# CESNET/UltraGrid

Measured on NVIDIA H100. Metric: 7680x4320 frames/sec encode (UYVY->DXT1), higher is better.
Workload: dtype f32

## Files before the change

include/ugb200.h:

```cpp
#ifndef UGB200_H
#define UGB200_H

#include "cuda_wrapper.h"

#ifdef __cplusplus
extern "C" {
#endif

enum ugb200_codec {
        UGB_VIDEO_CODEC_NONE = 0,
        UGB_RGBA, UGB_UYVY, UGB_YUYV, UGB_VUYA, UGB_R10k, UGB_R12L, UGB_v210, UGB_DVS10, UGB_DXT1, UGB_DXT1_YUV,
        UGB_DXT5, UGB_RGB, UGB_JPEG, UGB_JPEG_XS, UGB_RAW, UGB_H264, UGB_H265, UGB_VP8, UGB_VP9, UGB_BGR, UGB_J2K,
        UGB_J2KR, UGB_HW_VDPAU, UGB_HFYU, UGB_FFV1, UGB_CFHD, UGB_RG48, UGB_AV1, UGB_I420, UGB_Y216, UGB_Y416,
        UGB_PRORES, UGB_PRORES_4444, UGB_PRORES_4444_XQ, UGB_PRORES_422_HQ, UGB_PRORES_422, UGB_PRORES_422_PROXY,
        UGB_PRORES_422_LT, UGB_APV, UGB_PYROWAVE, UGB_DRM_PRIME,
        UGB_VIDEO_CODEC_COUNT
};


UGB_API int ugb200_rgb_to_dxt1_async(const void *src, void *out, int size_x, int size_y, cuda_wrapper_stream_t stream);
UGB_API int ugb200_yuv_to_dxt1_async(const void *src, void *out, int size_x, int size_y, cuda_wrapper_stream_t stream);
UGB_API int ugb200_rgb_to_dxt6_async(const void *src, void *out, int size_x, int size_y, cuda_wrapper_stream_t stream);
UGB_API int ugb200_yuv_to_dxt6_async(const void *src, void *out, int size_x, int size_y, cuda_wrapper_stream_t stream);

UGB_API int ugb200_uyvy_to_dxt1_async(const void *src, void *out, int size_x, int size_y, long src_pitch,
                              cuda_wrapper_stream_t stream);
UGB_API int ugb200_uyvy_to_dxt6_async(const void *src, void *out, int size_x, int size_y, long src_pitch,
                              cuda_wrapper_stream_t stream);

UGB_API int ugb200_pixfmt_supported(int in_codec, int out_codec);
UGB_API int ugb200_pixfmt_convert(int in_codec, int out_codec, void *dst, long dst_pitch, const void *src, long src_pitch,
                          int dst_len, int height, long src_size, int rshift, int gshift, int bshift,
                          cuda_wrapper_stream_t stream);

UGB_API int ugb200_pixfmt_staged_mode(int mode);

enum ugb200_line_func {
        UGB_LINE_ABGR_TO_RGB = 1,
        UGB_LINE_BGRA_TO_RGB,
        UGB_LINE_TO_RGBA_INPLACE,
        UGB_LINE_UYVY_TO_GRAYSCALE,
};
UGB_API int ugb200_vc_copyline(int func, void *dst, long dst_pitch, const void *src, long src_pitch, int dst_len, int height, long src_size,
                               int rshift, int gshift, int bshift, cuda_wrapper_stream_t stream);

UGB_API int ugb200_dxt1_to_rgb(const void *src, void *out, int w, int h, long out_pitch, int bgr, cuda_wrapper_stream_t stream);
UGB_API int ugb200_dxt5ycocg_to_rgb(const void *src, void *out, int w, int h, long out_pitch, int bgr, cuda_wrapper_stream_t stream);

struct ugb200_to_planar_data {
        int            width;
        int            height;
        unsigned char *out_data[4];
        unsigned       out_linesize[4];
        const unsigned char *in_data;
};
UGB_API int ugb200_v210_to_p010le(const struct ugb200_to_planar_data *d, long in_linesize, cuda_wrapper_stream_t stream);
UGB_API int ugb200_y216_to_p010le(const struct ugb200_to_planar_data *d, cuda_wrapper_stream_t stream);
UGB_API int ugb200_uyvy_to_nv12(const struct ugb200_to_planar_data *d, cuda_wrapper_stream_t stream);
UGB_API int ugb200_rgba_to_bgra(const struct ugb200_to_planar_data *d, cuda_wrapper_stream_t stream);
UGB_API int ugb200_vuya_to_i444(const struct ugb200_to_planar_data *d, cuda_wrapper_stream_t stream);
UGB_API int ugb200_uyvy_to_i420(const struct ugb200_to_planar_data *d, cuda_wrapper_stream_t stream);
UGB_API int ugb200_r12l_to_gbrp12le(const struct ugb200_to_planar_data *d, cuda_wrapper_stream_t stream);
UGB_API int ugb200_r12l_to_gbrp16le(const struct ugb200_to_planar_data *d, cuda_wrapper_stream_t stream);
UGB_API int ugb200_r12l_to_rgbp12le(const struct ugb200_to_planar_data *d, cuda_wrapper_stream_t stream);

struct ugb200_from_planar_data {
        int            width;
        int            height;
        unsigned char *out_data;
        unsigned       out_pitch;
        const unsigned char *in_data[4];
        unsigned       in_linesize[4];
        int            in_depth;
        int            log2_chroma_h;
        int            rgb_shift[3];
};
UGB_API int ugb200_gbrap_to_rgb(const struct ugb200_from_planar_data *d, cuda_wrapper_stream_t stream);
UGB_API int ugb200_gbrap_to_rgba(const struct ugb200_from_planar_data *d, cuda_wrapper_stream_t stream);
UGB_API int ugb200_gbrp10le_to_rgb(const struct ugb200_from_planar_data *d, cuda_wrapper_stream_t stream);
UGB_API int ugb200_gbrp12le_to_rgb(const struct ugb200_from_planar_data *d, cuda_wrapper_stream_t stream);
UGB_API int ugb200_gbrp16le_to_rgb(const struct ugb200_from_planar_data *d, cuda_wrapper_stream_t stream);
UGB_API int ugb200_rgbpXX_to_rgb(const struct ugb200_from_planar_data *d, cuda_wrapper_stream_t stream);
UGB_API int ugb200_gbrp10le_to_rgba(const struct ugb200_from_planar_data *d, cuda_wrapper_stream_t stream);
UGB_API int ugb200_gbrp12le_to_rgba(const struct ugb200_from_planar_data *d, cuda_wrapper_stream_t stream);
UGB_API int ugb200_gbrp16le_to_rgba(const struct ugb200_from_planar_data *d, cuda_wrapper_stream_t stream);
UGB_API int ugb200_gbrp10le_to_rg48(const struct ugb200_from_planar_data *d, cuda_wrapper_stream_t stream);
UGB_API int ugb200_gbrp12le_to_rg48(const struct ugb200_from_planar_data *d, cuda_wrapper_stream_t stream);
UGB_API int ugb200_gbrp16le_to_rg48(const struct ugb200_from_planar_data *d, cuda_wrapper_stream_t stream);
UGB_API int ugb200_rgbpXXle_to_rg48(const struct ugb200_from_planar_data *d, cuda_wrapper_stream_t stream);
UGB_API int ugb200_gbrp10le_to_r10k(const struct ugb200_from_planar_data *d, cuda_wrapper_stream_t stream);
UGB_API int ugb200_gbrp12le_to_r10k(const struct ugb200_from_planar_data *d, cuda_wrapper_stream_t stream);
UGB_API int ugb200_gbrp16le_to_r10k(const struct ugb200_from_planar_data *d, cuda_wrapper_stream_t stream);
UGB_API int ugb200_rgbpXXle_to_r10k(const struct ugb200_from_planar_data *d, cuda_wrapper_stream_t stream);
UGB_API int ugb200_gbrp12le_to_r12l(const struct ugb200_from_planar_data *d, cuda_wrapper_stream_t stream);
UGB_API int ugb200_gbrp16le_to_r12l(const struct ugb200_from_planar_data *d, cuda_wrapper_stream_t stream);
UGB_API int ugb200_rgbpXXle_to_r12l(const struct ugb200_from_planar_data *d, cuda_wrapper_stream_t stream);
UGB_API int ugb200_yuv444p_to_vuya(const struct ugb200_from_planar_data *d, cuda_wrapper_stream_t stream);
UGB_API int ugb200_yuv420p_to_uyvy(const struct ugb200_from_planar_data *d, cuda_wrapper_stream_t stream);
UGB_API int ugb200_yuv420_to_i420(const struct ugb200_from_planar_data *d, cuda_wrapper_stream_t stream);
UGB_API int ugb200_yuv422p_to_uyvy(const struct ugb200_from_planar_data *d, cuda_wrapper_stream_t stream);
UGB_API int ugb200_yuv422p_to_yuyv(const struct ugb200_from_planar_data *d, cuda_wrapper_stream_t stream);
UGB_API int ugb200_yuv422pXX_to_uyvy(const struct ugb200_from_planar_data *d, cuda_wrapper_stream_t stream);
UGB_API int ugb200_yuv422p10le_to_uyvy(const struct ugb200_from_planar_data *d, cuda_wrapper_stream_t stream);
UGB_API int ugb200_yuv422p10le_to_v210(const struct ugb200_from_planar_data *d, cuda_wrapper_stream_t stream);

#ifdef __cplusplus
}
#endif
#endif
```

ultragrid_b200/_lib.py:

```python
import ctypes
import os

_HERE = os.path.dirname(os.path.abspath(__file__))
LIB_PATH = os.path.join(_HERE, "libugb200.so")

_vp, _i, _l, _sz = ctypes.c_void_p, ctypes.c_int, ctypes.c_long, ctypes.c_size_t
SIGNATURES = {
    "cuda_rgb_to_dxt1": (_i, [_vp, _vp, _i, _i, _vp]),
    "cuda_yuv_to_dxt1": (_i, [_vp, _vp, _i, _i, _vp]),
    "cuda_rgb_to_dxt6": (_i, [_vp, _vp, _i, _i, _vp]),
    "cuda_yuv_to_dxt6": (_i, [_vp, _vp, _i, _i, _vp]),
    "cuda_yuv422_to_yuv444": (_i, [_vp, _vp, _i, _vp]),
    "cuda_wrapper_free": (_i, [_vp]),
    "cuda_wrapper_free_host": (_i, [_vp]),
    "cuda_wrapper_host_alloc": (_i, [ctypes.POINTER(_vp), _sz, ctypes.c_uint]),
    "cuda_wrapper_malloc": (_i, [ctypes.POINTER(_vp), _sz]),
    "cuda_wrapper_malloc_host": (_i, [ctypes.POINTER(_vp), _sz]),
    "cuda_wrapper_memcpy": (_i, [_vp, _vp, _sz, _i]),
    "cuda_wrapper_last_error_string": (ctypes.c_char_p, []),
    "cuda_wrapper_set_device": (_i, [_i]),
    "cuda_wrapper_get_last_error": (_i, []),
    "cuda_wrapper_get_error_string": (ctypes.c_char_p, [_i]),
    "cuda_wrapper_print_devices_info": (None, [ctypes.c_bool]),
    "cuda_wrapper_device_reset": (None, []),
    "cuda_wrapper_get_device_count": (_i, [ctypes.POINTER(_i)]),
    "cuda_wrapper_stream_create": (_i, [ctypes.POINTER(_vp)]),
    "cuda_wrapper_stream_destroy": (_i, [_vp]),
    "cuda_wrapper_stream_synchronize": (_i, [_vp]),
    "cuda_wrapper_memcpy_async": (_i, [_vp, _vp, _sz, _i, _vp]),
    "cuda_wrapper_memcpy2d": (_i, [_vp, _sz, _vp, _sz, _sz, _sz, _i]),
    "cuda_wrapper_device_numa_node": (_i, [_i]),
    "cuda_wrapper_bind_thread_to_device": (_i, [_i]),
    "cuda_wrapper_malloc_host_near": (_i, [ctypes.POINTER(_vp), _sz, _i]),
    "ugb200_rgb_to_dxt1_async": (_i, [_vp, _vp, _i, _i, _vp]),
    "ugb200_yuv_to_dxt1_async": (_i, [_vp, _vp, _i, _i, _vp]),
    "ugb200_rgb_to_dxt6_async": (_i, [_vp, _vp, _i, _i, _vp]),
    "ugb200_yuv_to_dxt6_async": (_i, [_vp, _vp, _i, _i, _vp]),
    "ugb200_uyvy_to_dxt1_async": (_i, [_vp, _vp, _i, _i, _l, _vp]),
    "ugb200_uyvy_to_dxt6_async": (_i, [_vp, _vp, _i, _i, _l, _vp]),
    "ugb200_dxt1_to_rgb": (_i, [_vp, _vp, _i, _i, _l, _i, _vp]),
    "ugb200_dxt5ycocg_to_rgb": (_i, [_vp, _vp, _i, _i, _l, _i, _vp]),
    "ugb200_vc_copyline": (_i, [_i, _vp, _l, _vp, _l, _i, _i, _l, _i, _i, _i, _vp]),
    "ugb200_pixfmt_supported": (_i, [_i, _i]),
    "ugb200_pixfmt_staged_mode": (_i, [_i]),
    "ugb200_pixfmt_convert": (_i, [_i, _i, _vp, _l, _vp, _l, _i, _i, _l, _i, _i, _i, _vp]),
    "ugb200_v210_to_p010le": (_i, [_vp, _l, _vp]),
    "ugb200_y216_to_p010le": (_i, [_vp, _vp]),
    "ugb200_uyvy_to_nv12": (_i, [_vp, _vp]),
    "ugb200_rgba_to_bgra": (_i, [_vp, _vp]),
    "ugb200_vuya_to_i444": (_i, [_vp, _vp]),
    "ugb200_uyvy_to_i420": (_i, [_vp, _vp]),
    "ugb200_r12l_to_gbrp12le": (_i, [_vp, _vp]),
    "ugb200_r12l_to_gbrp16le": (_i, [_vp, _vp]),
    "ugb200_r12l_to_rgbp12le": (_i, [_vp, _vp]),
    "ugb200_gbrap_to_rgb": (_i, [_vp, _vp]),
    "ugb200_gbrap_to_rgba": (_i, [_vp, _vp]),
    "ugb200_gbrp10le_to_rgb": (_i, [_vp, _vp]),
    "ugb200_gbrp12le_to_rgb": (_i, [_vp, _vp]),
    "ugb200_gbrp16le_to_rgb": (_i, [_vp, _vp]),
    "ugb200_rgbpXX_to_rgb": (_i, [_vp, _vp]),
    "ugb200_gbrp10le_to_rgba": (_i, [_vp, _vp]),
    "ugb200_gbrp12le_to_rgba": (_i, [_vp, _vp]),
    "ugb200_gbrp16le_to_rgba": (_i, [_vp, _vp]),
    "ugb200_gbrp10le_to_rg48": (_i, [_vp, _vp]),
    "ugb200_gbrp12le_to_rg48": (_i, [_vp, _vp]),
    "ugb200_gbrp16le_to_rg48": (_i, [_vp, _vp]),
    "ugb200_rgbpXXle_to_rg48": (_i, [_vp, _vp]),
    "ugb200_gbrp10le_to_r10k": (_i, [_vp, _vp]),
    "ugb200_gbrp12le_to_r10k": (_i, [_vp, _vp]),
    "ugb200_gbrp16le_to_r10k": (_i, [_vp, _vp]),
    "ugb200_rgbpXXle_to_r10k": (_i, [_vp, _vp]),
    "ugb200_gbrp12le_to_r12l": (_i, [_vp, _vp]),
    "ugb200_gbrp16le_to_r12l": (_i, [_vp, _vp]),
    "ugb200_rgbpXXle_to_r12l": (_i, [_vp, _vp]),
    "ugb200_yuv444p_to_vuya": (_i, [_vp, _vp]),
    "ugb200_yuv420p_to_uyvy": (_i, [_vp, _vp]),
    "ugb200_yuv420_to_i420": (_i, [_vp, _vp]),
    "ugb200_yuv422p_to_uyvy": (_i, [_vp, _vp]),
    "ugb200_yuv422p_to_yuyv": (_i, [_vp, _vp]),
    "ugb200_yuv422pXX_to_uyvy": (_i, [_vp, _vp]),
    "ugb200_yuv422p10le_to_uyvy": (_i, [_vp, _vp]),
    "ugb200_yuv422p10le_to_v210": (_i, [_vp, _vp]),
    "ugb200_jpeg_default_params": (None, [_vp]),
    "ugb200_jpeg_encoder_create": (_vp, [_vp]),
    "ugb200_jpeg_encoder_destroy": (None, [_vp]),
    "ugb200_jpeg_encode_device": (_i, [_vp, _vp, _l, _i, _i, _i, _vp]),
    "ugb200_jpeg_result_device": (_i, [_vp, ctypes.POINTER(_vp), ctypes.POINTER(_sz)]),
    "ugb200_jpeg_encode": (_i, [_vp, _vp, _i, _l, _i, _i, _i, _vp, ctypes.POINTER(_vp), ctypes.POINTER(_sz)]),
    "ugb200_jpeg_encode_into": (_i, [_vp, _vp, _i, _l, _i, _i, _i, _vp, _vp, _sz, ctypes.POINTER(_sz)]),
    "ugb200_jpeg_default_params_ex": (None, [_vp]),
    "ugb200_jpeg_encode_device_ex": (_i, [_vp, _vp, _l, _i, _i, _i, _vp]),
    "ugb200_jpeg_encode_into_ex": (_i, [_vp, _vp, _i, _l, _i, _i, _i, _vp, _vp, _sz, ctypes.POINTER(_sz)]),
    "ugb200_jpeg_encoder_stage_timing": (_i, [_vp, _i]),
    "ugb200_jpeg_encoder_stage_times": (_i, [_vp, ctypes.POINTER(ctypes.c_float)]),
    "ugb200_jpeg_get_image_info": (_i, [_vp, _sz, _vp]),
    "ugb200_jpeg_debug_segments": (_l, [_vp, _sz, _vp, _vp, _l]),
    "ugb200_jpeg_decoder_last_segments": (_l, [_vp, _vp, _vp, _l]),
    "ugb200_jpeg_decoder_create": (_vp, [_vp]),
    "ugb200_jpeg_decoder_destroy": (None, [_vp]),
    "ugb200_jpeg_decoder_expect": (_i, [_vp, _i, _i]),
    "ugb200_jpeg_decode": (_i, [_vp, _vp, _sz, _vp, _i, _l, _i, _i, _i, _i]),
    "ugb200_jpeg_debug_coefficients": (_i, [_vp, ctypes.POINTER(_vp), ctypes.POINTER(_sz)]),
    "ugb200_to_lavc_supported": (_i, [_i, _i]),
    "ugb200_to_lavc_convert": (_i, [_i, _i, _vp, _vp, _i, _i, _vp]),
    "ugb200_to_lavc_vid_conv_init": (_vp, [_i, _i, _i, _i]),
    "ugb200_to_lavc_vid_conv": (_vp, [_vp, _vp, _i]),
    "ugb200_to_lavc_vid_conv_destroy": (None, [_vp]),
    "ugb200_get_av_to_uv_conversion": (_vp, [_i, _i]),
    "ugb200_av_to_uv_convert": (_i, [_vp, _vp, _vp, _i, _i, _i, _vp, _vp]),
    "ugb200_av_to_uv_conversion_destroy": (None, [_vp]),
    "ugb200_set_cuda_devices": (_i, [ctypes.POINTER(_i), _i]),
    "ugb200_compress_init": (_vp, [ctypes.c_char_p]),
    "ugb200_compress_push": (_i, [_vp, _vp, _i, _i, _i, _i, ctypes.c_double]),
    "ugb200_compress_pop": (_i, [_vp, _vp, _sz, ctypes.POINTER(_sz), ctypes.POINTER(_i), ctypes.POINTER(ctypes.c_uint)]),
    "ugb200_compress_pop_ref": (_i, [_vp, ctypes.POINTER(_vp), ctypes.POINTER(_sz), ctypes.POINTER(_i), ctypes.POINTER(ctypes.c_uint)]),
    "ugb200_compress_done": (None, [_vp]),
    "ugb200_decompress_init": (_vp, [_i, _i]),
    "ugb200_decompress_module": (ctypes.c_char_p, [_vp]),
    "ugb200_decompress_reconfigure": (_i, [_vp, _i, _i, _i, _i, _i, _i, _i, _i]),
    "ugb200_decompress_frame": (_i, [_vp, _vp, _vp, ctypes.c_uint, _i, _vp]),
    "ugb200_decompress_done": (None, [_vp]),
    "ugb200_get_best_decoder_from": (_i, [_i, ctypes.POINTER(_i), _i]),
}

_lib = None


def load():
    global _lib
    if _lib is not None:
        return _lib
    if not os.path.exists(LIB_PATH):
        raise RuntimeError(
            f"{LIB_PATH} is missing: build it with `python -c 'import __graft_entry__ as g; g.build()'` "
            "(or `make -C ultragrid_b200/csrc`). There is no CPU fallback.")
    lib = ctypes.CDLL(LIB_PATH)
    for name, (res, args) in SIGNATURES.items():
        fn = getattr(lib, name)
        fn.restype = res
        fn.argtypes = args
    _lib = lib
    return lib
```

ultragrid_b200/csrc/dxt_kernels.cu:

```cuda
#include <cuda_runtime.h>
#include <stdint.h>
#include <stdlib.h>

#include "../../include/cuda_dxt.h"
#include "../../include/ugb200.h"
#include "dxt6_device.cuh"
#include "dxt_device.cuh"

namespace ugb {

__device__ __forceinline__ uint4 ld_stream_v4(const void *p)
{
        uint4 r;
        asm volatile("ld.global.nc.L1::no_allocate.v4.u32 {%0,%1,%2,%3}, [%4];"
                     : "=r"(r.x), "=r"(r.y), "=r"(r.z), "=r"(r.w)
                     : "l"(p));
        return r;
}
__device__ __forceinline__ uint2 ld_stream_v2(const void *p)
{
        uint2 r;
        asm volatile("ld.global.nc.L1::no_allocate.v2.u32 {%0,%1}, [%2];" : "=r"(r.x), "=r"(r.y) : "l"(p));
        return r;
}

template <int DXT_TYPE>
struct block_out;
template <>
struct block_out<1> {
        typedef uint2 type;
};
template <>
struct block_out<6> {
        typedef uint4 type;
};

template <int DXT_TYPE>
__device__ __forceinline__ typename block_out<DXT_TYPE>::type encode_block(const float (&r)[16], const float (&g)[16],
                                                                           const float (&b)[16]);
template <>
__device__ __forceinline__ uint2 encode_block<1>(const float (&r)[16], const float (&g)[16], const float (&b)[16])
{
        return dxt1_encode(r, g, b);
}
template <>
__device__ __forceinline__ uint4 encode_block<6>(const float (&r)[16], const float (&g)[16], const float (&b)[16])
{
        return dxt6_encode(r, g, b);
}

template <int DXT_TYPE>
struct uyvy_cta {
        static constexpr int threads = DXT_TYPE == 1 ? 64 : 128, min_ctas = DXT_TYPE == 1 ? 12 : 7;
};

template <int DXT_TYPE, int BPT, bool MIRROR>
__global__ void __launch_bounds__(uyvy_cta<DXT_TYPE>::threads, uyvy_cta<DXT_TYPE>::min_ctas) dxt_uyvy_kernel(const uint8_t *__restrict__ src, void *__restrict__ out,
                                                        int wb , int h, long pitch)
{
        typedef typename block_out<DXT_TYPE>::type out_t;
        const int gx = blockIdx.x * blockDim.x + threadIdx.x;
        const int by = blockIdx.y;
        if (gx >= wb / BPT) {
                return;
        }
        const int row0 = MIRROR ? h - 1 - by * 4 : by * 4;
        const uint8_t *p = src + (long) row0 * pitch + gx * (8 * BPT);
        const long step = MIRROR ? -pitch : pitch;

        uint32_t w[4][2 * BPT];
#pragma unroll
        for (int y = 0; y < 4; ++y, p += step) {
                if (BPT == 2) {
                        const uint4 v = ld_stream_v4(p);
                        w[y][0] = v.x, w[y][1] = v.y, w[y][2] = v.z, w[y][3] = v.w;
                } else {
                        const uint2 v = ld_stream_v2(p);
                        w[y][0] = v.x, w[y][1] = v.y;
                }
        }
        out_t *o = (out_t *) out + ((long) by * wb + gx * BPT);
        if constexpr (DXT_TYPE == 1 && BPT == 2) {
                const uint4 v[4] = { make_uint4(w[0][0], w[0][1], w[0][2], w[0][3]), make_uint4(w[1][0], w[1][1], w[1][2], w[1][3]),
                                     make_uint4(w[2][0], w[2][1], w[2][2], w[2][3]), make_uint4(w[3][0], w[3][1], w[3][2], w[3][3]) };
                *(uint4 *) o = dxt1_encode_uyvy_pair_skewed(v);
        } else {
#pragma unroll
                for (int k = 0; k < BPT; ++k) {
                        if constexpr (DXT_TYPE == 1) {
                                const uint32_t wk[4][2] = { { w[0][2 * k], w[0][2 * k + 1] }, { w[1][2 * k], w[1][2 * k + 1] },
                                                            { w[2][2 * k], w[2][2 * k + 1] }, { w[3][2 * k], w[3][2 * k + 1] } };
                                o[k] = dxt1_encode_uyvy_packed(wk);
                        } else {
                                float r[16], g[16], b[16];
#pragma unroll
                                for (int y = 0; y < 4; ++y) {
                                        load_row_uyvy_packed(w[y][2 * k], w[y][2 * k + 1], r + 4 * y, g + 4 * y, b + 4 * y);
                                }
                                o[k] = encode_block<DXT_TYPE>(r, g, b);
                        }
                }
        }
}

template <bool YUV, bool MIRROR, int DXT_TYPE>
__global__ void __launch_bounds__(128) dxt_packed3_kernel(const uint32_t *__restrict__ src, void *__restrict__ out,
                                                           int wb, int h)
{
        typedef typename block_out<DXT_TYPE>::type out_t;
        const int bx = blockIdx.x * blockDim.x + threadIdx.x;
        const int by = blockIdx.y;
        if (bx >= wb) {
                return;
        }
        const int stride_w = wb * 3;
        const int row0 = MIRROR ? h - 1 - by * 4 : by * 4;
        const uint32_t *p = src + ((long) stride_w * row0 + bx * 3);
        const int step = MIRROR ? -stride_w : stride_w;
        float r[16], g[16], b[16];
#pragma unroll
        for (int y = 0; y < 4; ++y, p += step) {
                load_row_packed3<YUV>(__ldg(p), __ldg(p + 1), __ldg(p + 2), r + 4 * y, g + 4 * y, b + 4 * y);
        }
        ((out_t *) out)[(long) by * wb + bx] = encode_block<DXT_TYPE>(r, g, b);
}

template <bool YUV, bool MIRROR>
__global__ void __launch_bounds__(64, 12) dxt1_packed3_pair_kernel(const uint8_t *__restrict__ src, void *__restrict__ out, int wb, int h)
{
        const int gx = blockIdx.x * blockDim.x + threadIdx.x;
        const int by = blockIdx.y;
        if (gx >= wb / 2) {
                return;
        }
        const long pitch = (long) wb * 12;
        const int row0 = MIRROR ? h - 1 - by * 4 : by * 4;
        const uint8_t *p = src + (long) row0 * pitch + (long) gx * 24;
        const long step = MIRROR ? -pitch : pitch;
        uint32_t wa[4][3], wb2[4][3];
#pragma unroll
        for (int y = 0; y < 4; ++y, p += step) {
                const uint2 q0 = ld_stream_v2(p), q1 = ld_stream_v2(p + 8), q2 = ld_stream_v2(p + 16);
                wa[y][0] = q0.x, wa[y][1] = q0.y, wa[y][2] = q1.x;
                wb2[y][0] = q1.y, wb2[y][1] = q2.x, wb2[y][2] = q2.y;
        }
        const uint2 ra = dxt1_encode_packed3<YUV>(wa), rb = dxt1_encode_packed3<YUV>(wb2);
        *((uint4 *) out + ((long) by * (wb / 2) + gx)) = make_uint4(ra.x, ra.y, rb.x, rb.y);
}

__global__ void __launch_bounds__(256) yuv422_to_yuv444_kernel(const uint4 *__restrict__ src, uint4 *__restrict__ out,
                                                                long groups16)
{
        const long gid = (long) blockIdx.x * blockDim.x + threadIdx.x;
        if (gid >= groups16) {
                return;
        }
        const uint4 a = ld_stream_v4(src + 2 * gid), c = ld_stream_v4(src + 2 * gid + 1);
        const uint32_t in[8] = { a.x, a.y, a.z, a.w, c.x, c.y, c.z, c.w };
        uint32_t o[12];
#pragma unroll
        for (int k = 0; k < 4; ++k) {
                const uint32_t p = in[2 * k], q = in[2 * k + 1];
                o[3 * k + 0] = __byte_perm(p, 0, 0x3201);
                o[3 * k + 1] = __byte_perm(p, q, 0x4520);
                o[3 * k + 2] = __byte_perm(q, 0, 0x2032);
        }
        out[3 * gid + 0] = make_uint4(o[0], o[1], o[2], o[3]);
        out[3 * gid + 1] = make_uint4(o[4], o[5], o[6], o[7]);
        out[3 * gid + 2] = make_uint4(o[8], o[9], o[10], o[11]);
}

__global__ void yuv422_to_yuv444_tail_kernel(const uint32_t *__restrict__ src, uint32_t *__restrict__ out, long first4,
                                             long groups4)
{
        const long gid = first4 + (long) blockIdx.x * blockDim.x + threadIdx.x;
        if (gid >= groups4) {
                return;
        }
        const uint32_t p = src[2 * gid], q = src[2 * gid + 1];
        out[3 * gid + 0] = __byte_perm(p, 0, 0x3201);
        out[3 * gid + 1] = __byte_perm(p, q, 0x4520);
        out[3 * gid + 2] = __byte_perm(q, 0, 0x2032);
}

template <bool YUV, int DXT_TYPE>
static int launch_packed3(const void *src, void *out, int sx, int sy, cudaStream_t str, bool sync)
{
        bool mirrored = false;
        if (sy < 0) {
                mirrored = true;
                sy = -sy;
        }
        if ((sx & 3) || (sy & 3) || (15 & (size_t) src) || (7 & (size_t) out) || (DXT_TYPE == 6 && (15 & (size_t) out))) {
                return -1;
        }
        const int wb = sx / 4, hb = sy / 4;
        if (hb > 65535) {
                return -1;
        }
        if (DXT_TYPE == 1 && wb > 0 && hb > 0 && !(wb & 1) && !(15 & (size_t) out)) {
                const dim3 grid((wb / 2 + 63) / 64, hb);
                if (mirrored) {
                        dxt1_packed3_pair_kernel<YUV, true><<<grid, 64, 0, str>>>((const uint8_t *) src, out, wb, sy);
                } else {
                        dxt1_packed3_pair_kernel<YUV, false><<<grid, 64, 0, str>>>((const uint8_t *) src, out, wb, sy);
                }
                if (cudaGetLastError() != cudaSuccess) {
                        return -2;
                }
        } else if (wb > 0 && hb > 0) {
                const int threads = 128;
                const dim3 grid((wb + threads - 1) / threads, hb);
                if (mirrored) {
                        dxt_packed3_kernel<YUV, true, DXT_TYPE><<<grid, threads, 0, str>>>((const uint32_t *) src, out, wb, sy);
                } else {
                        dxt_packed3_kernel<YUV, false, DXT_TYPE><<<grid, threads, 0, str>>>((const uint32_t *) src, out, wb, sy);
                }
                if (cudaGetLastError() != cudaSuccess) {
                        return -2;
                }
        }
        if (sync) {
                return cudaSuccess != cudaStreamSynchronize(str) ? -3 : 0;
        }
        return 0;
}

template <int DXT_TYPE>
static int launch_uyvy(const void *src, void *out, int sx, int sy, long pitch, cudaStream_t str)
{
        bool mirrored = false;
        if (sy < 0) {
                mirrored = true;
                sy = -sy;
        }
        if (pitch == 0) {
                pitch = (long) sx * 2;
        }
        const size_t out_align = DXT_TYPE == 6 ? 15 : 7;
        if ((sx & 3) || (sy & 3) || (7 & (size_t) src) || (out_align & (size_t) out) || (pitch & 7) || pitch < (long) sx * 2) {
                return -1;
        }
        const int wb = sx / 4, hb = sy / 4;
        if (wb == 0 || hb == 0) {
                return 0;
        }
        const int threads = uyvy_cta<DXT_TYPE>::threads;
        const bool pair = DXT_TYPE == 1 && !(wb & 1) && !(15 & (size_t) src) && !(pitch & 15) && !(15 & (size_t) out);
        if (hb > 65535) {
                return -1;
        }
        const int groups = pair ? wb / 2 : wb;
        const dim3 grid((groups + threads - 1) / threads, hb);
        const uint8_t *s = (const uint8_t *) src;
#define UGB_LAUNCH(BPT, MIR) dxt_uyvy_kernel<DXT_TYPE, BPT, MIR><<<grid, threads, 0, str>>>(s, out, wb, sy, pitch)
        if (DXT_TYPE == 1 && pair) {
                if constexpr (DXT_TYPE == 1) {
                        if (mirrored) {
                                UGB_LAUNCH(2, true);
                        } else {
                                UGB_LAUNCH(2, false);
                        }
                }
        } else {
                if (mirrored) {
                        UGB_LAUNCH(1, true);
                } else {
                        UGB_LAUNCH(1, false);
                }
        }
#undef UGB_LAUNCH
        return cudaGetLastError() != cudaSuccess ? -2 : 0;
}

}

extern "C" {

int cuda_rgb_to_dxt1(const void *src, void *out, int size_x, int size_y, cuda_wrapper_stream_t stream)
{
        return ugb::launch_packed3<false, 1>(src, out, size_x, size_y, (cudaStream_t) stream, true);
}
int cuda_yuv_to_dxt1(const void *src, void *out, int size_x, int size_y, cuda_wrapper_stream_t stream)
{
        return ugb::launch_packed3<true, 1>(src, out, size_x, size_y, (cudaStream_t) stream, true);
}
int cuda_rgb_to_dxt6(const void *src, void *out, int size_x, int size_y, cuda_wrapper_stream_t stream)
{
        return ugb::launch_packed3<false, 6>(src, out, size_x, size_y, (cudaStream_t) stream, true);
}
int cuda_yuv_to_dxt6(const void *src, void *out, int size_x, int size_y, cuda_wrapper_stream_t stream)
{
        return ugb::launch_packed3<true, 6>(src, out, size_x, size_y, (cudaStream_t) stream, true);
}

int cuda_yuv422_to_yuv444(const void *src, void *out, int pix_count, cuda_wrapper_stream_t str)
{
        cudaStream_t s = (cudaStream_t) str;
        if (pix_count < 0 || (3 & (size_t) src) || (3 & (size_t) out)) {
                return -1;
        }
        const long groups4 = pix_count / 4;
        long done4 = 0;
        if (!(15 & (size_t) src) && !(15 & (size_t) out)) {
                const long groups16 = groups4 / 4;
                if (groups16 > 0) {
                        ugb::yuv422_to_yuv444_kernel<<<(unsigned) ((groups16 + 255) / 256), 256, 0, s>>>(
                            (const uint4 *) src, (uint4 *) out, groups16);
                }
                done4 = groups16 * 4;
        }
        if (done4 < groups4) {
                const long rest = groups4 - done4;
                ugb::yuv422_to_yuv444_tail_kernel<<<(unsigned) ((rest + 255) / 256), 256, 0, s>>>(
                    (const uint32_t *) src, (uint32_t *) out, done4, groups4);
        }
        if (cudaGetLastError() != cudaSuccess) {
                return -2;
        }
        return cudaSuccess != cudaStreamSynchronize(s) ? -3 : 0;
}

int ugb200_rgb_to_dxt1_async(const void *src, void *out, int size_x, int size_y, cuda_wrapper_stream_t stream)
{
        return ugb::launch_packed3<false, 1>(src, out, size_x, size_y, (cudaStream_t) stream, false);
}
int ugb200_yuv_to_dxt1_async(const void *src, void *out, int size_x, int size_y, cuda_wrapper_stream_t stream)
{
        return ugb::launch_packed3<true, 1>(src, out, size_x, size_y, (cudaStream_t) stream, false);
}
int ugb200_rgb_to_dxt6_async(const void *src, void *out, int size_x, int size_y, cuda_wrapper_stream_t stream)
{
        return ugb::launch_packed3<false, 6>(src, out, size_x, size_y, (cudaStream_t) stream, false);
}
int ugb200_yuv_to_dxt6_async(const void *src, void *out, int size_x, int size_y, cuda_wrapper_stream_t stream)
{
        return ugb::launch_packed3<true, 6>(src, out, size_x, size_y, (cudaStream_t) stream, false);
}
int ugb200_uyvy_to_dxt1_async(const void *src, void *out, int size_x, int size_y, long src_pitch,
                              cuda_wrapper_stream_t stream)
{
        return ugb::launch_uyvy<1>(src, out, size_x, size_y, src_pitch, (cudaStream_t) stream);
}
int ugb200_uyvy_to_dxt6_async(const void *src, void *out, int size_x, int size_y, long src_pitch,
                              cuda_wrapper_stream_t stream)
{
        return ugb::launch_uyvy<6>(src, out, size_x, size_y, src_pitch, (cudaStream_t) stream);
}

}
```

Measured before the change: 16360.

## Overlap independent captured DXT1 encodes via programmatic dependent launch

After: 16630, median of 6. 1.6% higher.

```diff
diff --git a/include/ugb200.h b/include/ugb200.h
--- a/include/ugb200.h
+++ b/include/ugb200.h
@@ -27,6 +27,7 @@
                               cuda_wrapper_stream_t stream);
 UGB_API int ugb200_uyvy_to_dxt6_async(const void *src, void *out, int size_x, int size_y, long src_pitch,
                               cuda_wrapper_stream_t stream);
+UGB_API long ugb200_uyvy_to_dxt1_early_launches(void);
 
 UGB_API int ugb200_pixfmt_supported(int in_codec, int out_codec);
 UGB_API int ugb200_pixfmt_convert(int in_codec, int out_codec, void *dst, long dst_pitch, const void *src, long src_pitch,
diff --git a/ultragrid_b200/_lib.py b/ultragrid_b200/_lib.py
--- a/ultragrid_b200/_lib.py
+++ b/ultragrid_b200/_lib.py
@@ -38,6 +38,7 @@
     "ugb200_yuv_to_dxt6_async": (_i, [_vp, _vp, _i, _i, _vp]),
     "ugb200_uyvy_to_dxt1_async": (_i, [_vp, _vp, _i, _i, _l, _vp]),
     "ugb200_uyvy_to_dxt6_async": (_i, [_vp, _vp, _i, _i, _l, _vp]),
+    "ugb200_uyvy_to_dxt1_early_launches": (_l, []),
     "ugb200_dxt1_to_rgb": (_i, [_vp, _vp, _i, _i, _l, _i, _vp]),
     "ugb200_dxt5ycocg_to_rgb": (_i, [_vp, _vp, _i, _i, _l, _i, _vp]),
     "ugb200_vc_copyline": (_i, [_i, _vp, _l, _vp, _l, _i, _i, _l, _i, _i, _i, _vp]),
diff --git a/ultragrid_b200/csrc/dxt_kernels.cu b/ultragrid_b200/csrc/dxt_kernels.cu
--- a/ultragrid_b200/csrc/dxt_kernels.cu
+++ b/ultragrid_b200/csrc/dxt_kernels.cu
@@ -1,11 +1,16 @@
 #include <cuda_runtime.h>
 #include <stdint.h>
 #include <stdlib.h>
+
+#include <atomic>
+#include <mutex>
+#include <unordered_map>
 
 #include "../../include/cuda_dxt.h"
 #include "../../include/ugb200.h"
 #include "dxt6_device.cuh"
 #include "dxt_device.cuh"
+#include "dxt_overlap.h"
 
 namespace ugb {
 
@@ -59,6 +64,9 @@
                                                         int wb , int h, long pitch)
 {
         typedef typename block_out<DXT_TYPE>::type out_t;
+        if constexpr (DXT_TYPE == 1) {
+                asm volatile("griddepcontrol.launch_dependents;");
+        }
         const int gx = blockIdx.x * blockDim.x + threadIdx.x;
         const int by = blockIdx.y;
         if (gx >= wb / BPT) {
@@ -101,6 +109,9 @@
                         }
                 }
         }
+        if constexpr (DXT_TYPE == 1) {
+                asm volatile("griddepcontrol.wait;" ::: "memory");
+        }
 }
 
 template <bool YUV, bool MIRROR, int DXT_TYPE>
@@ -226,6 +237,43 @@
         return 0;
 }
 
+static std::mutex dxt1_chains_mu;
+static std::unordered_map<cudaStream_t, overlap_chain> dxt1_chains;
+static std::atomic<long> dxt1_early_launches{ 0 };
+
+static int launch_dxt1(void (*kernel)(const uint8_t *, void *, int, int, long), dim3 grid, cudaStream_t str, const uint8_t *s, void *out,
+                       int wb, int sy, long pitch, const encode_io &io)
+{
+        cudaStreamCaptureStatus st = cudaStreamCaptureStatusNone;
+        unsigned long long id = 0;
+        const cudaGraphNode_t *deps = nullptr;
+        size_t ndeps = 0;
+        if (str == nullptr || str == cudaStreamLegacy || cudaStreamGetCaptureInfo(str, &st, &id, nullptr, &deps, &ndeps) != cudaSuccess ||
+            st != cudaStreamCaptureStatusActive) {
+                kernel<<<grid, uyvy_cta<1>::threads, 0, str>>>(s, out, wb, sy, pitch);
+                return cudaGetLastError() != cudaSuccess ? -2 : 0;
+        }
+        std::lock_guard<std::mutex> lock(dxt1_chains_mu);
+        overlap_chain &chain = dxt1_chains[str];
+        const bool early = chain.admits(id, (const void *const *) deps, ndeps, io);
+        cudaLaunchAttribute attr[1];
+        attr[0].id = cudaLaunchAttributeProgrammaticStreamSerialization;
+        attr[0].val.programmaticStreamSerializationAllowed = 1;
+        cudaLaunchConfig_t cfg = {};
+        cfg.gridDim = grid, cfg.blockDim = dim3(uyvy_cta<1>::threads), cfg.dynamicSmemBytes = 0, cfg.stream = str;
+        cfg.attrs = attr, cfg.numAttrs = early ? 1 : 0;
+        if (cudaLaunchKernelEx(&cfg, kernel, s, out, wb, sy, pitch) != cudaSuccess ||
+            cudaStreamGetCaptureInfo(str, &st, &id, nullptr, &deps, &ndeps) != cudaSuccess || ndeps != 1) {
+                chain = overlap_chain();
+                return cudaGetLastError() != cudaSuccess ? -2 : 0;
+        }
+        chain.push(id, deps[0], early, io);
+        if (early) {
+                ++dxt1_early_launches;
+        }
+        return 0;
+}
+
 template <int DXT_TYPE>
 static int launch_uyvy(const void *src, void *out, int sx, int sy, long pitch, cudaStream_t str)
 {
@@ -253,23 +301,18 @@
         const int groups = pair ? wb / 2 : wb;
         const dim3 grid((groups + threads - 1) / threads, hb);
         const uint8_t *s = (const uint8_t *) src;
-#define UGB_LAUNCH(BPT, MIR) dxt_uyvy_kernel<DXT_TYPE, BPT, MIR><<<grid, threads, 0, str>>>(s, out, wb, sy, pitch)
-        if (DXT_TYPE == 1 && pair) {
-                if constexpr (DXT_TYPE == 1) {
-                        if (mirrored) {
-                                UGB_LAUNCH(2, true);
-                        } else {
-                                UGB_LAUNCH(2, false);
-                        }
-                }
+        if constexpr (DXT_TYPE == 1) {
+                const uintptr_t s0 = (uintptr_t) s, o0 = (uintptr_t) out;
+                const encode_io io = { { s0, s0 + (uintptr_t) ((long) (sy - 1) * pitch + (long) sx * 2) }, { o0, o0 + (uintptr_t) wb * hb * 8 } };
+                return launch_dxt1(pair ? (mirrored ? dxt_uyvy_kernel<1, 2, true> : dxt_uyvy_kernel<1, 2, false>)
+                                        : (mirrored ? dxt_uyvy_kernel<1, 1, true> : dxt_uyvy_kernel<1, 1, false>),
+                                   grid, str, s, out, wb, sy, pitch, io);
+        }
+        if (mirrored) {
+                dxt_uyvy_kernel<DXT_TYPE, 1, true><<<grid, threads, 0, str>>>(s, out, wb, sy, pitch);
         } else {
-                if (mirrored) {
-                        UGB_LAUNCH(1, true);
-                } else {
-                        UGB_LAUNCH(1, false);
-                }
-        }
-#undef UGB_LAUNCH
+                dxt_uyvy_kernel<DXT_TYPE, 1, false><<<grid, threads, 0, str>>>(s, out, wb, sy, pitch);
+        }
         return cudaGetLastError() != cudaSuccess ? -2 : 0;
 }
 
@@ -347,5 +390,9 @@
 {
         return ugb::launch_uyvy<6>(src, out, size_x, size_y, src_pitch, (cudaStream_t) stream);
 }
-
-}
+long ugb200_uyvy_to_dxt1_early_launches(void)
+{
+        return ugb::dxt1_early_launches.load();
+}
+
+}
diff --git a/ultragrid_b200/csrc/dxt_overlap.h b/ultragrid_b200/csrc/dxt_overlap.h
--- /dev/null
+++ b/ultragrid_b200/csrc/dxt_overlap.h
@@ -0,0 +1,56 @@
+#pragma once
+
+#include <stddef.h>
+#include <stdint.h>
+
+namespace ugb {
+
+struct byte_range {
+        uintptr_t lo, hi;
+};
+
+inline bool ranges_meet(byte_range a, byte_range b)
+{
+        return a.lo < b.hi && b.lo < a.hi;
+}
+
+struct encode_io {
+        byte_range src, out;
+};
+
+inline bool independent(const encode_io &a, const encode_io &b)
+{
+        return !ranges_meet(a.out, b.src) && !ranges_meet(a.src, b.out) && !ranges_meet(a.out, b.out);
+}
+
+struct overlap_chain {
+        static constexpr int max_len = 64;
+        unsigned long long capture_id = 0;
+        const void *tail = nullptr;
+        int len = 0;
+        encode_io io[max_len];
+
+        bool admits(unsigned long long id, const void *const *deps, size_t ndeps, const encode_io &next) const
+        {
+                if (id == 0 || id != capture_id || ndeps != 1 || deps[0] != tail || len == 0 || len >= max_len) {
+                        return false;
+                }
+                for (int i = 0; i < len; ++i) {
+                        if (!independent(io[i], next)) {
+                                return false;
+                        }
+                }
+                return true;
+        }
+
+        void push(unsigned long long id, const void *node, bool early, const encode_io &launched)
+        {
+                if (!early) {
+                        len = 0;
+                }
+                capture_id = id, tail = node;
+                io[len++] = launched;
+        }
+};
+
+}
```
